# welcomyou/sherpa-vietnamese-asr

Hardware: AMD Instinct MI355X
Metric: audio-sec/sec (xRT) Zipformer-68M offline decode (higher is better)
Workload: dtype bf16; 1 GPU; zipformer-68m greedy_search, batched planner chunks, 1 h per GPU; model=zipformer-68m, weights=greedy-calibrated, chunks_per_gpu=121, batch_pipeline=True, encoder_frames_per_gpu=98813

## Files before the change

include/zasr.h:

```cpp
#ifndef ZASR_H_
#define ZASR_H_

#include <stdint.h>

#ifdef __cplusplus
extern "C" {
#endif

typedef struct zasr_recognizer zasr_recognizer;
typedef struct zasr_result zasr_result;

enum {
  ZASR_OK = 0,
  ZASR_ERR_INVALID = 1,
  ZASR_ERR_NOT_FOUND = 2,
  ZASR_ERR_RUNTIME = 3,
};

enum {
  ZASR_PRECISION_FP32 = 0,
  ZASR_PRECISION_BF16 = 1,
  ZASR_PRECISION_BF16_ENC = 2,
  ZASR_PRECISION_BF16X3 = 3,
  ZASR_PRECISION_BF16X6 = 4,
// ... 107 lines not shown
int zasr_vad_probs(zasr_vad* h, const float* audio, const int64_t* offsets,
                   const int64_t* lengths, int32_t n_files, int32_t auto_boost, float* probs);
int zasr_vad_probs_device(zasr_vad* h, const float* d_audio, const int64_t* offsets,
                          const int64_t* lengths, int32_t n_files, int32_t auto_boost,
                          float* d_probs, void* stream);
int32_t zasr_vad_last_passes(const zasr_vad* h);
int zasr_vad_window(zasr_vad* h, const float* input, const float* state, int32_t n, float* prob,
                    float* state_out);

int32_t zasr_vocab_size(const zasr_recognizer* h);
int32_t zasr_joiner_dim(const zasr_recognizer* h);
int zasr_model_routes(zasr_recognizer* h, char* buf, int64_t cap);
int zasr_fbank_set_mel_banks(zasr_recognizer* h, const float* banks, int32_t n_bins);
int zasr_selftest_launch(int32_t block_threads);
int zasr_selftest_gemm_h3r(int32_t M, int32_t K, int32_t N, int32_t epi, const float* A,
                           const float* W, const float* bias, float* C);
int zasr_selftest_ffn_h3(int32_t R, int32_t D, int32_t F, const float* Y, const float* W1,
                         const float* b1, const float* W2, const float* b2,
                         const float* byp_orig, const float* byp_scale, float* X);
int zasr_selftest_ffn_bf16(int32_t R, int32_t D, int32_t F, const float* W1, const float* b1,
                           const float* W2, const float* b2, const float* byp_orig,
                           const float* byp_scale, float* X, int32_t form);
int zasr_selftest_ffn_bf16_oop(int32_t R, int32_t D, int32_t F, const float* W1, const float* b1,
                               const float* W2, const float* b2, const float* byp_orig,
                               const float* byp_scale, float* X, float* Xout, int32_t form);
int zasr_selftest_ffn_h3_oop(int32_t R, int32_t D, int32_t F, const float* W1, const float* b1,
                             const float* W2, const float* b2, const float* byp_orig,
                             const float* byp_scale, float* X, float* Xout);
int zasr_selftest_seam(int32_t nseq, const int32_t* L, int32_t d, int32_t ds, int32_t dn,
                       int32_t ds_next, int32_t c0, int32_t ldo, const float* xd,
                       const float* orig, const float* s, const float* wn8, const float* wo2,
                       float* next, float* xnext, float* out, float* next_ref, float* xnext_ref,
                       float* out_ref);
int zasr_selftest_attn_block_map(const int32_t* lens, int32_t nseq, int32_t units_per_seq,
                                 int32_t order, uint32_t* out, int64_t cap, int32_t* grid);

int zasr_profile_enable(zasr_recognizer* h, int32_t on);
int zasr_profile_reset(zasr_recognizer* h);
int zasr_profile_report(zasr_recognizer* h, char* buf, int64_t cap);

const char* zasr_last_error(void);
const char* zasr_version(void);

#ifdef __cplusplus
}
#endif
#endif
```

sherpa-vietnamese-asr_amd/csrc/engine.cpp:

```cpp
#include "engine.h"

#include <algorithm>
#include <cmath>
#include <cstring>
#include <deque>
#include <numeric>
#include <cstdlib>
#include <sstream>

#include "common.h"
#include "gemm.h"
#include "host_io.h"
#include "onnx_io.h"

namespace zasr {

namespace {
struct HwNode {
  int tok = -1;
  double tok_score = 0, node_score = 0, out_score = 0;
  bool is_end = false;
  std::vector<std::pair<int, int>> kids;
  int fail = 0, out = -1;
  int child(int t) const {
// ... 583 lines not shown
        for (DLin* l : {&L.na_in, &L.na_out}) mk(*l);
        for (int a = 0; a < 2; ++a)
          for (DLin* l : {&L.sa_in[a], &L.sa_out[a], &L.cv_in[a], &L.cv_out[a]}) mk(*l);
        for (int a = 0; a < 3; ++a)
          for (DLin* l : {&L.ff_in[a], &L.ff_out[a]}) mk(*l);
      }
    ZASR_HIP_CHECK(hipStreamSynchronize(stream_));
    for (DLin* l : {&model_.pw1, &model_.pw2}) {
      std::vector<__bf16> h((size_t)l->N * l->K), pk(h.size());
      ZASR_HIP_CHECK(hipMemcpy(h.data(), l->wh, h.size() * 2, hipMemcpyDeviceToHost));
      pack_frag32_host(h.data(), l->N, l->K, pk.data());
      void* p = nullptr;
      ZASR_HIP_CHECK(hipMalloc(&p, pk.size() * 2));
      model_.allocations.push_back(p);
      ZASR_HIP_CHECK(hipMemcpy(p, pk.data(), pk.size() * 2, hipMemcpyHostToDevice));
      l->wp = p;
    }
    for (auto& s : model_.stacks)
      for (auto& L : s.layers)
        for (int a = 0; a < 3; ++a) {
          const int F = L.ff_in[a].N, d = L.ff_in[a].K;
          if (d < 256 || !ffn_fused_supported(d) || F % 32 != 0 || F > 2048) continue;
          for (DLin* l : {&L.ff_in[a], &L.ff_out[a]}) {
            std::vector<__bf16> h((size_t)l->N * l->K), pk(h.size());
            ZASR_HIP_CHECK(hipMemcpy(h.data(), l->wh, h.size() * 2, hipMemcpyDeviceToHost));
            ffn_pack_host(h.data(), l->N, l->K, pk.data());
            void* p = nullptr;
            ZASR_HIP_CHECK(hipMalloc(&p, pk.size() * 2));
            model_.allocations.push_back(p);
            ZASR_HIP_CHECK(hipMemcpy(p, pk.data(), pk.size() * 2, hipMemcpyHostToDevice));
            l->wp = p;
          }
        }
  }
  {
    const double gb = (double)cfg.V * cfg.V * cfg.joiner_dim * 4.0 / 1e9;
    double max_gb = 24.0;
    if (const char* e = getenv("ZASR_DEC_TABLE_MAX_GB")) max_gb = atof(e);
    if (gb <= max_gb) {
      void* p = nullptr;
      ZASR_HIP_CHECK(hipMalloc(&p, (size_t)cfg.V * cfg.V * cfg.joiner_dim * sizeof(float)));
      model_.allocations.push_back(p);
      model_.dec_table = reinterpret_cast<float*>(p);
      DecoderW dw{model_.dec_tap0, model_.dec_tap1, model_.dec_proj.b, cfg.joiner_dim};
      launch_dec_table(dw, model_.dec_proj.w, cfg.V, model_.dec_table, stream_);
      ZASR_HIP_CHECK(hipStreamSynchronize(stream_));
    }
  }

  {
    std::vector<double> tw(512);
    for (int j = 0; j < 256; ++j) {
      double a = -2.0 * M_PI * j / 512.0;
      tw[2 * j] = std::cos(a);
      tw[2 * j + 1] = std::sin(a);
    }
    ZASR_HIP_CHECK(hipMalloc(&d_twiddle_, 512 * sizeof(double)));
    ZASR_HIP_CHECK(hipMemcpy(d_twiddle_, tw.data(), 512 * sizeof(double), hipMemcpyHostToDevice));
    std::vector<float> win(400);
    for (int i = 0; i < 400; ++i)
      win[i] = (float)std::pow(0.5 - 0.5 * std::cos(2.0 * M_PI / 399.0 * i), 0.85);
    d_window_ = dev(win.data(), 400);
    auto mel = [](float f) { return 1127.0f * logf(1.0f + f / 700.0f); };
    const float mlo = mel(20.0f), mhi = mel(7600.0f);
    const float delta = (mhi - mlo) / 81.0f;
    std::vector<float> banks(80 * 256, 0.f);
// ... 427 lines not shown
      a.v = vv;
      a.out = oa;
      a.map = bm.heads;
      a.map_len = bm.n_heads;
      prof_begin("attn_apply");
      launch_attn_flash(a, k == 0 ? 1 : 2, st_);
      prof_end();
      linear_h(Ly.sa_out[k], oa, true, 12 * h, R, X, false, d, EPI_RESADD);
      return;
    }
    float* vv = ws<float>("ly_vv", (size_t)R * 12 * h);
    float* oa = ws<float>("ly_oa", (size_t)R * 12 * h);
    linear(Ly.sa_in[k], X, d, R, vv, 12 * h, EPI_NONE);
    if (np) {
      AttnFlashArgs a = fa;
      a.v = vv;
      a.out = oa;
      a.map = bm.heads;
      a.map_len = bm.n_heads;
      prof_begin("attn_apply");
      launch_attn_flash(a, k == 0 ? 1 : 2, st_);
      prof_end();
      linear(Ly.sa_out[k], oa, 12 * h, R, X, d, EPI_RESADD);
      return;
    }
    AttnSAArgs sa{qkp, h, Ly.pos_tab, model_.pmax, d_off, B, maxL, stats, vv, oa, stats};
    prof_begin("attn_apply");
    launch_attn_sa(sa, k == 0, false, st_);
    prof_end();
    linear(Ly.sa_out[k], oa, 12 * h, R, X, d, EPI_RESADD);
  };
  auto conv = [&](int k) {
    if (Ly.cv_in[k].wh) {
      __bf16* dc = ws<__bf16>("ly_dc_h", (size_t)R * d);
      if (Ly.cv_in[k].glu) {
        __bf16* g = ws<__bf16>("ly_glu_h", (size_t)R * d);
        linear_h(Ly.cv_in[k], X, false, d, R, g, true, d, EPI_GLU);
        prof_begin("dwconv1d");
        launch_dwconv1d_post_glu_bf16(g, d_off, d_map, R, d, S.K, Ly.cv_dw_w[k], Ly.cv_dw_b[k], dc, st_);
        prof_end();
      } else {
        __bf16* g2 = ws<__bf16>("ly_g2_h", (size_t)R * 2 * d);
        linear_h(Ly.cv_in[k], X, false, d, R, g2, true, 2 * d, EPI_NONE);
        prof_begin("dwconv1d");
        launch_glu_dwconv1d_bf16(g2, d_off, d_map, R, d, S.K, Ly.cv_dw_w[k], Ly.cv_dw_b[k], dc, st_);
        prof_end();
      }
      linear_h(Ly.cv_out[k], dc, true, d, R, X, false, d, EPI_RESADD);
      return;
    }
    float* dc = ws<float>("ly_dc", (size_t)R * d);
    if (Ly.cv_in[k].glu) {
      float* g = ws<float>("ly_glu", (size_t)R * d);
      linear(Ly.cv_in[k], X, d, R, g, d, EPI_GLU);
      prof_begin("dwconv1d");
      launch_dwconv1d_post_glu(g, d_off, d_map, R, d, S.K, Ly.cv_dw_w[k], Ly.cv_dw_b[k], dc, st_);
      prof_end();
    } else {
      float* g2 = ws<float>("ly_g2", (size_t)R * 2 * d);
      linear(Ly.cv_in[k], X, d, R, g2, 2 * d, EPI_NONE);
      prof_begin("dwconv1d");
      launch_glu_dwconv1d(g2, d_off, d_map, R, d, S.K, Ly.cv_dw_w[k], Ly.cv_dw_b[k], dc, st_);
      prof_end();
    }
    linear(Ly.cv_out[k], dc, d, R, X, d, EPI_RESADD);
  };
// ... 1084 lines not shown
```

sherpa-vietnamese-asr_amd/csrc/kernels.h:

```cpp
#pragma once
#include <cstdint>
#include <vector>

#include <hip/hip_runtime.h>

namespace zasr {

struct FbankTables {
  const double* twiddle;
  const float* window;
  const int* mel_start;
  const int* mel_len;
  const int* mel_woff;
  const float* mel_w;
};
void launch_fbank(const float* wav, const long* wav_off, const int* nsamp, const int* fr_off,
                  int nseq, int total_frames, const FbankTables& tabs, float* out,
                  hipStream_t st, bool campp = false);

void launch_silence_flags(const float* wav, long n, int frame_len, float threshold,
                          unsigned char* flags, hipStream_t st);

void launch_selftest_noop(int block_threads);
void selftest_gemm_h3r(int M, int K, int N, int epi, const float* A, const float* W,
// ... 101 lines not shown
                  int total_rows, const float* w , const float* b, void* out,
                  bool out_bf16, hipStream_t st, bool fast = false);
void pack_frag32_host(const __bf16* w, int rows, int cols, __bf16* out);
void launch_convnext_bf16(const void* x, const int* L_off, const int* L_map, int total_rows,
                          const float* dw_w, const float* dw_b, const void* w1, const float* b1,
                          const void* w2, const float* b2, void* ytmp, void* out,
                          hipStream_t st);
void launch_convnext_mlp_h3(const float* y, const float* x, long npos, const void* w1p,
                            const float* b1, const void* w2p, const float* b2, float* out,
                            hipStream_t st);
void launch_dwconv2d_tiled(const float* x, const int* L_off, const int* L_map, int total_rows,
                           const float* w, const float* b, float* out, hipStream_t st);

void selftest_seam(int nseq, const int* L, int d, int ds, int dn, int ds_next, int c0, int ldo,
                   const float* xd, const float* orig, const float* s, const float* wn8,
                   const float* wo2, float* next, float* xnext, float* out, float* next_ref,
                   float* xnext_ref, float* out_ref);
void launch_bias_norm(float* x, int rows, int d, const float* bias, float log_scale,
                      const float* orig, const float* bypass_scale, hipStream_t st,
                      float* copy_out = nullptr);
void launch_bypass(float* x, const float* orig, const float* s, long rows, int d, hipStream_t st);
void launch_glu(const float* x2, float* g, long rows, int d, hipStream_t st);
void launch_dwconv1d_post_glu(const float* g, const int* off, const int* map, int total_rows,
                              int d, int K, const float* w, const float* b, float* out,
                              hipStream_t st);
void launch_dwconv1d_post_glu_bf16(const void* g, const int* off, const int* map,
                                   int total_rows, int d, int K, const float* w, const float* b,
                                   void* out, hipStream_t st);
void launch_glu_dwconv1d(const float* x2, const int* off, const int* map, int total_rows, int d,
                         int K, const float* w, const float* b, float* out, hipStream_t st);
void launch_glu_dwconv1d_bf16(const void* x2, const int* off, const int* map, int total_rows,
                              int d, int K, const float* w, const float* b, void* out,
                              hipStream_t st);
void launch_nonlin_prep(const float* h3, float* t1, long rows, int hid, hipStream_t st);
void launch_downsample(const float* x, const int* off_in, const int* off_out, const int* map_out,
                       int total_out, int d, int ds, const float* w_host8, float* out,
                       hipStream_t st);
void launch_upsample_combine(const float* xd, const float* orig, const int* off_in,
                             const int* off_ds, const int* map_in, int total_rows, int d, int ds,
                             const float* s, float* y, hipStream_t st);
void launch_stack_glue(const float* xd, const float* orig, const int* off_in, const int* off_ds,
                       const int* map_in, int rows, int d, int ds, const float* s, float* next,
                       int dn, float* full, int ldf, int c0, hipStream_t st);
struct SeamDesc {
  const float* xd = nullptr;
  const float* orig = nullptr;
  const float* s = nullptr;
  const int* off_in = nullptr;
  const int* off_ds = nullptr;
  const int* off_run = nullptr;
  const int* map_run = nullptr;
  int runs = 0;
  int rows = 0;
  int d = 0, ds = 1;
  float* next = nullptr;
  int dn = 0;
  int ds_next = 1;
  float* xnext = nullptr;
  const float* wn_host8 = nullptr;
  float* out = nullptr;
  const int* off_out = nullptr;
  const float* wo_host2 = nullptr;
  int ldo = 0, c0 = 0;
};
void launch_seam(const SeamDesc& s, hipStream_t st);
void launch_row2seq(const int* off, int nseq, int total, int* map, hipStream_t st);
// ... 230 lines not shown
```

sherpa-vietnamese-asr_amd/csrc/selftest.cpp:

```cpp
#include <cstring>
#include <memory>
#include <vector>

#include "common.h"
#include "gemm.h"
#include "kernels.h"

namespace zasr {
namespace {
struct DevBuf {
  void* p = nullptr;
  explicit DevBuf(size_t bytes) { ZASR_HIP_CHECK(hipMalloc(&p, bytes > 0 ? bytes : 4)); }
  ~DevBuf() { (void)hipFree(p); }
  template <class T>
  T* as() const { return reinterpret_cast<T*>(p); }
};
void up(DevBuf& d, const void* h, size_t bytes) {
  if (bytes) ZASR_HIP_CHECK(hipMemcpy(d.p, h, bytes, hipMemcpyHostToDevice));
}
}

void selftest_gemm_h3r(int M, int K, int N, int epi, const float* A, const float* W,
                       const float* bias, float* C) {
  ZASR_REQUIRE(M >= 1, "selftest gemm_h3r: M >= 1");
// ... 160 lines not shown
    sd.wn_host8 = wn8;
  }
  if (has_out) {
    sd.out = dout.as<float>();
    sd.off_out = dO.as<int>();
    sd.wo_host2 = wo2;
    sd.ldo = ldo;
    sd.c0 = c0;
  }
  launch_seam(sd, nullptr);
  launch_stack_glue(dxd.as<float>(), dorig.as<float>(), dL.as<int>(), dS.as<int>(), mL.as<int>(),
                    rows, d, ds, ds_.as<float>(), dn > 0 ? dnext_r.as<float>() : nullptr, dn,
                    has_out ? dfull.as<float>() : nullptr, ldo, c0, nullptr);
  if (has_x)
    launch_downsample(dnext_r.as<float>(), dL.as<int>(), dN.as<int>(), mN.as<int>(), rn, dn,
                      ds_next, wn8, dxn_r.as<float>(), nullptr);
  if (has_out)
    launch_downsample(dfull.as<float>(), dL.as<int>(), dO.as<int>(), mO.as<int>(), ro, ldo, 2, wo2,
                      dout_r.as<float>(), nullptr);
  ZASR_HIP_CHECK(hipDeviceSynchronize());
  auto down = [](void* h, const DevBuf& dv, size_t bytes) {
    if (bytes) ZASR_HIP_CHECK(hipMemcpy(h, dv.p, bytes, hipMemcpyDeviceToHost));
  };
  down(next, dnext, bn);
  down(next_ref, dnext_r, bn);
  if (has_x) {
    down(xnext, dxn, bxn);
    down(xnext_ref, dxn_r, bxn);
  }
  down(out, dout, bout);
  down(out_ref, dout_r, bout);
}

}
```

sherpa-vietnamese-asr_amd/csrc/zasr_api.cpp:

```cpp
#include <cstdio>
#include <cstring>
#include <fstream>
#include <memory>
#include <mutex>
#include <sstream>
#include <string>
#include <vector>

#include "../../include/zasr.h"
#include "campp.h"
#include "common.h"
#include "vad.h"
#include "vibert.h"
#include "engine.h"
#include "host_io.h"
#include "onnx_io.h"

using zasr::Engine;
using zasr::TokenResult;

struct zasr_recognizer {
  std::unique_ptr<Engine> eng;
  std::string model_dir;
  std::string tokens_path;
// ... 660 lines not shown
                               const float* byp_scale, float* X, float* Xout, int32_t form) {
  if (!W1 || !b1 || !W2 || !b2 || !X || !Xout) return fail(ZASR_ERR_INVALID, "null argument");
  return guarded([&]() {
    zasr::selftest_ffn_bf16(R, D, F, W1, b1, W2, b2, byp_orig, byp_scale, X, form, Xout);
    return (int)ZASR_OK;
  });
}

int zasr_selftest_ffn_h3_oop(int32_t R, int32_t D, int32_t F, const float* W1, const float* b1,
                             const float* W2, const float* b2, const float* byp_orig,
                             const float* byp_scale, float* X, float* Xout) {
  if (!W1 || !b1 || !W2 || !b2 || !X || !Xout) return fail(ZASR_ERR_INVALID, "null argument");
  return guarded([&]() {
    zasr::selftest_ffn_h3(R, D, F, nullptr, W1, b1, W2, b2, byp_orig, byp_scale, X, Xout);
    return (int)ZASR_OK;
  });
}

int zasr_selftest_seam(int32_t nseq, const int32_t* L, int32_t d, int32_t ds, int32_t dn,
                       int32_t ds_next, int32_t c0, int32_t ldo, const float* xd,
                       const float* orig, const float* s, const float* wn8, const float* wo2,
                       float* next, float* xnext, float* out, float* next_ref, float* xnext_ref,
                       float* out_ref) {
  if (!L || !orig || !wn8 || !wo2 || !next || !xnext || !out || !next_ref || !xnext_ref ||
      !out_ref || (ds > 1 && (!xd || !s)))
    return fail(ZASR_ERR_INVALID, "null argument");
  return guarded([&]() {
    zasr::selftest_seam(nseq, L, d, ds, dn, ds_next, c0, ldo, xd, orig, s, wn8, wo2, next, xnext,
                        out, next_ref, xnext_ref, out_ref);
    return (int)ZASR_OK;
  });
}

int zasr_selftest_attn_block_map(const int32_t* lens, int32_t nseq, int32_t units_per_seq,
                                 int32_t order, uint32_t* out, int64_t cap, int32_t* grid) {
  if (!lens || !grid || (cap > 0 && !out) || cap < 0) return fail(ZASR_ERR_INVALID, "null argument");
  return guarded([&]() {
    std::vector<unsigned> map;
    *grid = zasr::build_attn_block_map(lens, nseq, units_per_seq, order, map);
    if ((int64_t)map.size() > cap) return fail(ZASR_ERR_INVALID, "block map buffer too small");
    std::copy(map.begin(), map.end(), out);
    return (int)ZASR_OK;
  });
}

int zasr_silence_flags(const float* d_wav, int64_t n, int32_t frame_len, float threshold,
                       uint8_t* d_flags, void* stream) {
  if (n < 0 || (n > 0 && (!d_wav || !d_flags))) return fail(ZASR_ERR_INVALID, "null argument");
  return guarded([&]() {
    zasr::launch_silence_flags(d_wav, (long)n, (int)frame_len, threshold, d_flags,
                               reinterpret_cast<hipStream_t>(stream));
    return (int)ZASR_OK;
  });
}

int zasr_set_tokens(zasr_recognizer* h, const char* tokens_path) {
  if (!h || !tokens_path) return fail(ZASR_ERR_INVALID, "null argument");
  return guarded([&]() {
    std::ifstream f(tokens_path);
    if (!f) return fail(ZASR_ERR_NOT_FOUND, std::string("tokens file not found: ") + tokens_path);
    std::lock_guard<std::mutex> lk(h->sym_mu);
    h->tokens_path = tokens_path;
    h->syms.reset();
    return (int)ZASR_OK;
  });
}
// ... 100 lines not shown
```

sherpa-vietnamese-asr_amd/zasr/binding.py:

```python
from __future__ import annotations

import ctypes as C
import dataclasses
import os
from typing import List, Optional, Sequence

import numpy as np

_PKG = os.path.dirname(os.path.dirname(os.path.abspath(__file__)))
DEFAULT_LIB = os.path.join(_PKG, "lib", "libzasr.so")

EXPORTS = (
    "zasr_create", "zasr_destroy", "zasr_convert_model", "zasr_convert_stage_model", "zasr_fbank", "zasr_decode_batch", "zasr_decode_features",
    "zasr_decode_device", "zasr_decode_device_batches", "zasr_encode_features", "zasr_search_encoder_out",
    "zasr_result_count", "zasr_result_num_tokens", "zasr_result_num_frames",
    "zasr_result_tokens", "zasr_result_frames", "zasr_result_log_probs",
    "zasr_result_token_stats", "zasr_result_free", "zasr_vocab_size", "zasr_joiner_dim",
    "zasr_profile_enable", "zasr_profile_reset", "zasr_profile_report", "zasr_last_error",
    "zasr_version", "zasr_campp_create", "zasr_campp_destroy", "zasr_campp_embedding_dim",
    "zasr_campp_fbank", "zasr_campp_embed", "zasr_campp_embed_device", "zasr_campp_windows_device",
    "zasr_vibert_create", "zasr_vibert_destroy", "zasr_vibert_num_labels",
    "zasr_vibert_num_detect", "zasr_vibert_run",
    "zasr_vad_create", "zasr_vad_destroy", "zasr_vad_probs", "zasr_vad_probs_device",
    "zasr_vad_window", "zasr_vad_last_passes", "zasr_silence_flags",
    "zasr_create_stream", "zasr_destroy_stream", "zasr_stream_accept_waveform",
    "zasr_decode_stream", "zasr_decode_streams", "zasr_stream_is_decoded",
    "zasr_stream_num_tokens", "zasr_stream_num_frames", "zasr_stream_tokens",
    "zasr_stream_frames", "zasr_stream_log_probs", "zasr_stream_token_stats",
    "zasr_stream_result_json", "zasr_set_tokens", "zasr_model_routes",
    "zasr_fbank_set_mel_banks", "zasr_selftest_launch", "zasr_decode_host_batches",
    "zasr_selftest_gemm_h3r", "zasr_selftest_ffn_h3", "zasr_selftest_ffn_bf16",
    "zasr_selftest_attn_block_map", "zasr_selftest_seam", "zasr_selftest_ffn_bf16_oop",
    "zasr_selftest_ffn_h3_oop",
)


PRECISIONS = {"fp32": 0, "bf16": 1, "bf16_enc": 2, "bf16x3": 3, "bf16x6": 4, "f16x3": 5}


C_FP = C.POINTER(C.c_float)


class ZasrError(RuntimeError):
    pass


class _Config(C.Structure):
    _fields_ = [
        ("model_dir", C.c_char_p),
        ("decoding_method", C.c_char_p),
        ("max_active_paths", C.c_int32),
        ("blank_penalty", C.c_float),
        ("hotword_tokens", C.POINTER(C.c_int32)),
        ("hotword_lens", C.POINTER(C.c_int32)),
        ("hotword_scores", C.POINTER(C.c_float)),
        ("num_hotwords", C.c_int32),
        ("device_id", C.c_int32),
        ("precision", C.c_int32),
    ]


_lib = None


def load_library(path: Optional[str] = None) -> C.CDLL:
    global _lib
# ... 121 lines not shown
    lib.zasr_stream_tokens.argtypes = [P]
    lib.zasr_stream_tokens.restype = C.POINTER(I32)
    lib.zasr_stream_frames.argtypes = [P]
    lib.zasr_stream_frames.restype = C.POINTER(I32)
    lib.zasr_stream_log_probs.argtypes = [P]
    lib.zasr_stream_log_probs.restype = C.POINTER(C.c_double)
    lib.zasr_stream_token_stats.argtypes = [P]
    lib.zasr_stream_token_stats.restype = fp
    lib.zasr_stream_result_json.argtypes = [P, C.c_char_p, I64, C.POINTER(I64)]
    lib.zasr_stream_result_json.restype = C.c_int
    lib.zasr_set_tokens.argtypes = [P, C.c_char_p]
    lib.zasr_set_tokens.restype = C.c_int
    lib.zasr_model_routes.argtypes = [P, C.c_char_p, I64]
    lib.zasr_model_routes.restype = C.c_int
    lib.zasr_fbank_set_mel_banks.argtypes = [P, fp, I32]
    lib.zasr_fbank_set_mel_banks.restype = C.c_int
    lib.zasr_selftest_launch.argtypes = [I32]
    lib.zasr_selftest_launch.restype = C.c_int
    lib.zasr_selftest_gemm_h3r.argtypes = [I32, I32, I32, I32, fp, fp, fp, fp]
    lib.zasr_selftest_gemm_h3r.restype = C.c_int
    lib.zasr_selftest_ffn_h3.argtypes = [I32, I32, I32, fp, fp, fp, fp, fp, fp, fp, fp]
    lib.zasr_selftest_ffn_h3.restype = C.c_int
    lib.zasr_selftest_ffn_bf16.argtypes = [I32, I32, I32, fp, fp, fp, fp, fp, fp, fp, I32]
    lib.zasr_selftest_ffn_bf16.restype = C.c_int
    lib.zasr_selftest_attn_block_map.argtypes = [C.POINTER(I32), I32, I32, I32,
                                                 C.POINTER(C.c_uint32), I64, C.POINTER(I32)]
    lib.zasr_selftest_attn_block_map.restype = C.c_int
    lib.zasr_selftest_seam.argtypes = [I32, C.POINTER(I32)] + [I32] * 6 + [fp] * 11
    lib.zasr_selftest_seam.restype = C.c_int
    lib.zasr_selftest_ffn_bf16_oop.argtypes = [I32, I32, I32] + [fp] * 8 + [I32]
    lib.zasr_selftest_ffn_bf16_oop.restype = C.c_int
    lib.zasr_selftest_ffn_h3_oop.argtypes = [I32, I32, I32] + [fp] * 8
    lib.zasr_selftest_ffn_h3_oop.restype = C.c_int
    if path is None:
        _lib = lib
    return lib


def convert_model(model_dir: str, out_dir: str, lib_path: Optional[str] = None) -> None:
    lib = load_library(lib_path)
    os.makedirs(out_dir, exist_ok=True)
    rc = lib.zasr_convert_model(model_dir.encode(), out_dir.encode())
    if rc != 0:
        msg = lib.zasr_last_error().decode()
        if rc == 2:
            raise FileNotFoundError(msg)
        raise ZasrError(msg)


def convert_stage_model(kind: str, model_dir: str, out_dir: str,
                        lib_path: Optional[str] = None) -> None:
    lib = load_library(lib_path)
    os.makedirs(out_dir, exist_ok=True)
    rc = lib.zasr_convert_stage_model(kind.encode(), model_dir.encode(), out_dir.encode())
    if rc != 0:
        msg = lib.zasr_last_error().decode()
        if rc == 2:
            raise FileNotFoundError(msg)
        raise ZasrError(msg)


def selftest_launch(block_threads: int, lib_path: Optional[str] = None) -> None:
    lib = load_library(lib_path)
    rc = lib.zasr_selftest_launch(int(block_threads))
    if rc != 0:
        raise ZasrError(lib.zasr_last_error().decode())
# ... 70 lines not shown
            p(out))
    if kind == "bf16":
        rc = lib.zasr_selftest_ffn_bf16_oop(*args, int(form))
    elif kind == "h3":
        rc = lib.zasr_selftest_ffn_h3_oop(*args)
    else:
        raise ValueError(kind)
    if rc != 0:
        raise ZasrError(lib.zasr_last_error().decode())
    return out, X


def selftest_seam(L, d: int, ds: int, dn: int, ds_next: int, c0: int, ldo: int, xd, orig, s,
                  wn8, wo2, fill: float = -777.25, lib_path: Optional[str] = None) -> dict:
    lib = load_library(lib_path)
    L = np.ascontiguousarray(L, dtype=np.int32)
    orig, wn8, wo2 = _f32(orig), _f32(wn8), _f32(wo2)
    xd = None if xd is None else _f32(xd)
    s = None if s is None else _f32(s)
    rows = int(L.sum())
    rn = int(((L + ds_next - 1) // ds_next).sum())
    ro = int(((L + 1) // 2).sum())
    assert orig.shape == (rows, d) and wn8.shape == (8,) and wo2.shape == (2,)
    assert ds == 1 or (xd.shape == (int(((L + ds - 1) // ds).sum()), d) and s.shape == (d,))
    res = {}
    for name, shape in (("next", (rows, dn)), ("xnext", (rn, dn)), ("out", (ro, ldo))):
        for k in (name, name + "_ref"):
            res[k] = np.full(shape, fill, dtype=np.float32)
    p = lambda x: None if x is None else x.ctypes.data_as(C_FP)
    rc = lib.zasr_selftest_seam(len(L), L.ctypes.data_as(C.POINTER(C.c_int32)), int(d), int(ds),
                                int(dn), int(ds_next), int(c0), int(ldo), p(xd), p(orig), p(s),
                                p(wn8), p(wo2), p(res["next"]), p(res["xnext"]), p(res["out"]),
                                p(res["next_ref"]), p(res["xnext_ref"]), p(res["out_ref"]))
    if rc != 0:
        raise ZasrError(lib.zasr_last_error().decode())
    return res


def silence_flags(d_wav_ptr: int, n: int, frame_len: int, threshold: float, d_flags_ptr: int,
                  stream: int = 0, lib_path: Optional[str] = None) -> None:
    lib = load_library(lib_path)
    rc = lib.zasr_silence_flags(C.c_void_p(d_wav_ptr), int(n), int(frame_len),
                                float(threshold), C.c_void_p(d_flags_ptr), C.c_void_p(stream))
    if rc != 0:
        raise ZasrError(lib.zasr_last_error().decode())


@dataclasses.dataclass
class SearchResult:
    token_ids: np.ndarray
    frames: np.ndarray
    log_probs: np.ndarray
    stats: np.ndarray
    T: int


def _f32(a) -> np.ndarray:
    return np.ascontiguousarray(np.asarray(a, dtype=np.float32))


def _ptr_array(arrs: Sequence[np.ndarray]):
    fp = C.POINTER(C.c_float)
    return (fp * len(arrs))(*[a.ctypes.data_as(fp) for a in arrs])


class Recognizer:
# ... 431 lines not shown
```

Measured before the change: 134,800 audio-sec/sec.

## Fuse depthwise conv, SwooshR and conv output GEMM into one conv-tail kernel

Adds a kernel that computes the depthwise 1D convolution with SwooshR activation per 64-row tile in LDS, then immediately feeds that tile to MFMA to do the output projection with bias and residual add into X. This removes the round trip of writing and re-reading the intermediate bf16 activation, along with one kernel launch per conv module. It is enabled only for d=192, K=31 layers that use the GLU input path, with output weights repacked into MFMA fragment order at load. The cost is a more complex kernel with boundary masking across sequence edges and possibly lower occupancy than the tuned standalone GEMM.

Result: no change. 135,400 audio-sec/sec (median of 6 runs) (+0.5%).

```diff
diff --git a/include/zasr.h b/include/zasr.h
--- a/include/zasr.h
+++ b/include/zasr.h
@@ -163,6 +163,11 @@
                        const float* orig, const float* s, const float* wn8, const float* wo2,
                        float* next, float* xnext, float* out, float* next_ref, float* xnext_ref,
                        float* out_ref);
+int zasr_selftest_conv_tail(int32_t nseq, const int32_t* lens, int32_t d, int32_t K,
+                            const float* g, const float* dw_w, const float* dw_b, const float* W,
+                            const float* b, const float* X_in, float* X_pair_out,
+                            float* X_fused_out, int32_t pad_rows, float* g_after);
+int zasr_conv_tail_supported(int32_t d, int32_t K);
 int zasr_selftest_attn_block_map(const int32_t* lens, int32_t nseq, int32_t units_per_seq,
                                  int32_t order, uint32_t* out, int64_t cap, int32_t* grid);
 
diff --git a/sherpa-vietnamese-asr_amd/csrc/conv_tail.hip b/sherpa-vietnamese-asr_amd/csrc/conv_tail.hip
--- /dev/null
+++ b/sherpa-vietnamese-asr_amd/csrc/conv_tail.hip
@@ -0,0 +1,293 @@
+#include "common.h"
+#include "gemm_dev.h"
+#include "kernels.h"
+
+namespace zasr {
+
+namespace {
+
+constexpr int kCtRows = 64;
+constexpr int kCtLdc = 72;
+constexpr int kCtLde = 40;
+
+__device__ __forceinline__ void ct_lds_barrier() {
+  asm volatile("s_waitcnt lgkmcnt(0)" ::: "memory");
+  __builtin_amdgcn_s_barrier();
+}
+
+template <int D, int K>
+__global__ __launch_bounds__(256, 2) void conv_tail_kernel(
+    const __bf16* __restrict__ g, const int* __restrict__ off, const int* __restrict__ map,
+    int total_rows, const float* __restrict__ w, const float* __restrict__ bias,
+    const __bf16* __restrict__ Wp, const float* __restrict__ b_out, float* __restrict__ X) {
+  constexpr int half = K / 2;
+  constexpr int nrows = kCtRows + K - 1;
+  constexpr int NG = D / 64;
+  constexpr int nvec = nrows * 8;
+  constexpr int kIt = (nvec + 255) / 256;
+  constexpr int nw4 = 16 * K;
+  constexpr int kWIt = (nw4 + 255) / 256;
+  static_assert(kWIt <= 2, "conv_tail: two tap vectors per thread");
+  constexpr int WM = D == 192 ? 2 : 1, WN = 4 / WM;
+  constexpr int WTM = kCtRows / WM, WTN = D / WN;
+  constexpr int FM = WTM / 32, FN = WTN / 32;
+  static_assert(D % 64 == 0 && WTN % 32 == 0 && FM >= 1 && FN >= 1, "conv_tail: tile split");
+  constexpr int WH = FN >= 3 ? 2 : 4;
+  static_assert(WH == 2 || WH == 4, "conv_tail: one or two fragment batches per chunk");
+  constexpr int NF = FM * FN;
+  constexpr int PD = NF < 4 ? NF : 4;
+  constexpr int tileB = nrows * 64 * 2;
+  constexpr int epiB = 4 * 32 * kCtLde * 4;
+  constexpr int tileBytes = 2 * tileB > epiB ? 2 * tileB : epiB;
+  __shared__ __attribute__((aligned(16))) unsigned char tileRaw[tileBytes];
+  __shared__ __attribute__((aligned(16))) float sW[2][64 * K];
+  __shared__ __attribute__((aligned(16))) __bf16 sDC[2][kCtRows * kCtLdc];
+  __shared__ int sLo[kCtRows], sHi[kCtRows], sMasked;
+  unsigned short* const tile16 = reinterpret_cast<unsigned short*>(tileRaw);
+
+  const int r0 = xcd_tile(blockIdx.x, gridDim.x) * kCtRows;
+  const int tid = threadIdx.x, lane = tid & 63, wid = tid >> 6;
+  const int wm = wid / WN, wn = wid - wm * WN;
+  const int c = lane;
+  if (tid == 0) sMasked = 0;
+
+  bf16x8 gv[kIt];
+  float4 wv0, wv1;
+  float bnext;
+  auto gload = [&](int gi) {
+    const int c0 = gi * 64;
+#pragma unroll
+    for (int q = 0; q < kIt; ++q) {
+      const int e = tid + 256 * q;
+      const int c8 = e & 7, rr = e >> 3;
+      int r = r0 - half + rr;
+      r = r < 0 ? 0 : (r >= total_rows ? total_rows - 1 : r);
+      gv[q] = *reinterpret_cast<const bf16x8*>(g + (long)r * D + c0 + 8 * c8);
+    }
+    const float4* w4 = reinterpret_cast<const float4*>(w + (long)c0 * K);
+    wv0 = w4[tid < nw4 ? tid : nw4 - 1];
+    if constexpr (kWIt > 1) wv1 = w4[tid + 256 < nw4 ? tid + 256 : nw4 - 1];
+    bnext = bias[c0 + c];
+  };
+  auto sstore = [&](int buf) {
+    unsigned short* t = tile16 + buf * (nrows * 64);
+#pragma unroll
+    for (int q = 0; q < kIt; ++q) {
+      const int e = tid + 256 * q;
+      const int c8 = e & 7, rr = e >> 3;
+      const int r = r0 - half + rr;
+      bf16x8 v = gv[q];
+      if (r < 0 || r >= total_rows) {
+#pragma unroll
+        for (int j = 0; j < 8; ++j) v[j] = (__bf16)0.f;
+      }
+      if (e < nvec) *reinterpret_cast<bf16x8*>(&t[rr * 64 + 8 * c8]) = v;
+    }
+    if (tid < nw4) *reinterpret_cast<float4*>(&sW[buf][4 * tid]) = wv0;
+    if constexpr (kWIt > 1) {
+      if (tid + 256 < nw4) *reinterpret_cast<float4*>(&sW[buf][4 * (tid + 256)]) = wv1;
+    }
+  };
+
+  gload(0);
+  int seq_lo = 0, seq_hi = 0;
+  if (tid < kCtRows && r0 + tid < total_rows) {
+    const int b = map[r0 + tid];
+    seq_lo = off[b];
+    seq_hi = off[b + 1];
+  }
+  sstore(0);
+  float bc = bnext;
+  if (tid < kCtRows) {
+    const int r = r0 + tid;
+    int lo = -half, hi = half;
+    if (r < total_rows) {
+      lo = max(seq_lo - r, -half);
+      hi = min(seq_hi - 1 - r, half);
+    }
+    sLo[tid] = lo;
+    sHi[tid] = hi;
+    if (lo != -half || hi != half) atomicOr(&sMasked, 1);
+  }
+  __syncthreads();
+  const bool masked = sMasked != 0;
+  const int tr0 = wid * 16;
+
+  f32x16 acc[FM][FN];
+#pragma unroll
+  for (int i = 0; i < FM; ++i)
+#pragma unroll
+    for (int j = 0; j < FN; ++j)
+#pragma unroll
+      for (int r = 0; r < 16; ++r) acc[i][j][r] = 0.f;
+
+  const bf16x8* Wf = reinterpret_cast<const bf16x8*>(Wp) + (long)(wn * FN) * (D / 16) * 64 + lane;
+  bf16x8 bw[WH][FN];
+  auto wload = [&](int ks0) {
+#pragma unroll
+    for (int s = 0; s < WH; ++s)
+#pragma unroll
+      for (int j = 0; j < FN; ++j) bw[s][j] = Wf[((long)j * (D / 16) + ks0 + s) * 64];
+  };
+  auto mma = [&](const __bf16* dc, int s0) {
+#pragma unroll
+    for (int s = 0; s < WH; ++s) {
+      bf16x8 a[FM];
+#pragma unroll
+      for (int i = 0; i < FM; ++i)
+        a[i] = *reinterpret_cast<const bf16x8*>(
+            &dc[(wm * WTM + i * 32 + (lane & 31)) * kCtLdc + (s0 + s) * 16 + 8 * (lane >> 5)]);
+#pragma unroll
+      for (int i = 0; i < FM; ++i)
+#pragma unroll
+        for (int j = 0; j < FN; ++j)
+          acc[i][j] = __builtin_amdgcn_mfma_f32_32x32x16_bf16(a[i], bw[s][j], acc[i][j], 0, 0, 0);
+    }
+  };
+
+  for (int gi = 0; gi < NG; ++gi) {
+    const int buf = gi & 1;
+    gload(gi + 1 < NG ? gi + 1 : NG - 1);
+    wload(gi * 4);
+    const unsigned short* t = tile16 + buf * (nrows * 64);
+    auto tv = [&](int rr) {
+      return __builtin_bit_cast(float, (unsigned)t[(tr0 + rr) * 64 + c] << 16);
+    };
+    float wr[K];
+#pragma unroll
+    for (int k = 0; k < K; ++k) wr[k] = sW[buf][c * K + k];
+    float cacc[16];
+#pragma unroll
+    for (int i = 0; i < 16; ++i) cacc[i] = bc;
+    if (!masked) {
+#pragma unroll
+      for (int rr = 0; rr < 16 + K - 1; ++rr) {
+        const float v = tv(rr);
+#pragma unroll
+        for (int i = 0; i < 16; ++i) {
+          const int k = rr - i;
+          if (k >= 0 && k < K) cacc[i] = fmaf(wr[k], v, cacc[i]);
+        }
+      }
+    } else {
+      int lo[16], hi[16];
+#pragma unroll
+      for (int i = 0; i < 16; ++i) {
+        lo[i] = __builtin_amdgcn_readfirstlane(sLo[tr0 + i]);
+        hi[i] = __builtin_amdgcn_readfirstlane(sHi[tr0 + i]);
+      }
+#pragma unroll
+      for (int rr = 0; rr < 16 + K - 1; ++rr) {
+        const float v = tv(rr);
+#pragma unroll
+        for (int i = 0; i < 16; ++i) {
+          const int k = rr - i;
+          if (k >= 0 && k < K && k - half >= lo[i] && k - half <= hi[i])
+            cacc[i] = fmaf(wr[k], v, cacc[i]);
+        }
+      }
+    }
+    __bf16* dc = sDC[buf];
+#pragma unroll
+    for (int i = 0; i < 16; ++i) dc[(tr0 + i) * kCtLdc + c] = (__bf16)swooshr_fast(cacc[i]);
+    if (gi + 1 < NG) {
+      sstore(buf ^ 1);
+      bc = bnext;
+    }
+    ct_lds_barrier();
+    mma(dc, 0);
+    if constexpr (WH < 4) {
+      wload(gi * 4 + WH);
+      mma(dc, WH);
+    }
+  }
+  asm volatile("s_waitcnt vmcnt(0)" ::: "memory");
+
+  float* sE = reinterpret_cast<float*>(tileRaw) + wid * (32 * kCtLde);
+  const int c4 = lane & 7;
+  auto xload = [&](int f, float4 (&pre)[4]) {
+    const int i = f / FN, j = f - i * FN;
+    const int col = wn * WTN + j * 32 + 4 * c4;
+#pragma unroll
+    for (int q = 0; q < 4; ++q) {
+      const int row = r0 + wm * WTM + i * 32 + (lane >> 3) + 8 * q;
+      pre[q] = *reinterpret_cast<const float4*>(
+          X + (long)(row < total_rows ? row : total_rows - 1) * D + col);
+    }
+  };
+  float4 pre[PD][4];
+#pragma unroll
+  for (int f = 0; f < PD; ++f) xload(f, pre[f]);
+#pragma unroll
+  for (int f = 0; f < NF; ++f) {
+    const int i = f / FN, j = f - i * FN;
+#pragma unroll
+    for (int r = 0; r < 16; ++r)
+      sE[((r & 3) + 8 * (r >> 2) + 4 * (lane >> 5)) * kCtLde + (lane & 31)] = acc[i][j][r];
+    __builtin_amdgcn_wave_barrier();
+    const int col = wn * WTN + j * 32 + 4 * c4;
+    float4 bo = make_float4(0.f, 0.f, 0.f, 0.f);
+    if (b_out) bo = *reinterpret_cast<const float4*>(b_out + col);
+    float4 o[4];
+#pragma unroll
+    for (int q = 0; q < 4; ++q) o[q] = pre[f % PD][q];
+    if (f + PD < NF) xload(f + PD, pre[f % PD]);
+#pragma unroll
+    for (int q = 0; q < 4; ++q) {
+      const int rl = (lane >> 3) + 8 * q;
+      const int row = r0 + wm * WTM + i * 32 + rl;
+      float4 v = *reinterpret_cast<const float4*>(&sE[rl * kCtLde + 4 * c4]);
+      if (row < total_rows) {
+        v.x = fmaf(v.x, 1.f, bo.x) + o[q].x;
+        v.y = fmaf(v.y, 1.f, bo.y) + o[q].y;
+        v.z = fmaf(v.z, 1.f, bo.z) + o[q].z;
+        v.w = fmaf(v.w, 1.f, bo.w) + o[q].w;
+        *reinterpret_cast<float4*>(X + (long)row * D + col) = v;
+      }
+    }
+    __builtin_amdgcn_wave_barrier();
+  }
+}
+
+}
+
+bool conv_tail_instantiated(int d, int K) {
+  return (K == 31 && (d == 192 || d == 256)) || (K == 15 && (d == 256 || d == 384 || d == 512));
+}
+
+bool conv_tail_supported(int d, int K) { return d == 192 && K == 31; }
+
+void conv_tail_pack_host(const __bf16* w, int d, __bf16* out) {
+  for (int nf = 0; nf < d / 32; ++nf)
+    for (int ks = 0; ks < d / 16; ++ks)
+      for (int l = 0; l < 64; ++l)
+        for (int j = 0; j < 8; ++j)
+          out[(((size_t)nf * (d / 16) + ks) * 64 + l) * 8 + j] =
+              w[(size_t)(32 * nf + (l & 31)) * d + 16 * ks + 8 * (l >> 5) + j];
+}
+
+void launch_conv_tail(const void* g, const int* off, const int* map, int total_rows, int d, int Kr,
+                      const float* dw_w, const float* dw_b, const void* W_out_packed,
+                      const float* b_out, float* X, hipStream_t st) {
+  if (total_rows <= 0) return;
+  ZASR_REQUIRE(conv_tail_instantiated(d, Kr), "conv_tail: no kernel for (channels, kernel size)");
+  ZASR_REQUIRE((reinterpret_cast<uintptr_t>(g) & 15) == 0 && (reinterpret_cast<uintptr_t>(dw_w) & 15) == 0 &&
+                   (reinterpret_cast<uintptr_t>(W_out_packed) & 15) == 0 &&
+                   (reinterpret_cast<uintptr_t>(X) & 15) == 0 &&
+                   (b_out == nullptr || (reinterpret_cast<uintptr_t>(b_out) & 15) == 0),
+               "conv_tail: operands must be 16-byte aligned");
+  const __bf16* gh = reinterpret_cast<const __bf16*>(g);
+  const __bf16* wp = reinterpret_cast<const __bf16*>(W_out_packed);
+  const dim3 grid(cdiv(total_rows, kCtRows));
+#define ZASR_CT(D_, K_)                                                                      \
+  ZASR_LAUNCH((conv_tail_kernel<D_, K_>), grid, dim3(256), 0, st, gh, off, map, total_rows, \
+              dw_w, dw_b, wp, b_out, X)
+  if (d == 192) ZASR_CT(192, 31);
+  else if (d == 256 && Kr == 31) ZASR_CT(256, 31);
+  else if (d == 256) ZASR_CT(256, 15);
+  else if (d == 384) ZASR_CT(384, 15);
+  else ZASR_CT(512, 15);
+#undef ZASR_CT
+}
+
+}
diff --git a/sherpa-vietnamese-asr_amd/csrc/engine.cpp b/sherpa-vietnamese-asr_amd/csrc/engine.cpp
--- a/sherpa-vietnamese-asr_amd/csrc/engine.cpp
+++ b/sherpa-vietnamese-asr_amd/csrc/engine.cpp
@@ -639,6 +639,20 @@
             l->wp = p;
           }
         }
+    for (auto& s : model_.stacks)
+      for (auto& L : s.layers)
+        for (int a = 0; a < 2; ++a) {
+          DLin& l = L.cv_out[a];
+          if (!L.cv_in[a].glu || l.N != s.d || l.K != s.d || !conv_tail_supported(s.d, s.K)) continue;
+          std::vector<__bf16> h((size_t)l.N * l.K), pk(h.size());
+          ZASR_HIP_CHECK(hipMemcpy(h.data(), l.wh, h.size() * 2, hipMemcpyDeviceToHost));
+          conv_tail_pack_host(h.data(), s.d, pk.data());
+          void* p = nullptr;
+          ZASR_HIP_CHECK(hipMalloc(&p, pk.size() * 2));
+          model_.allocations.push_back(p);
+          ZASR_HIP_CHECK(hipMemcpy(p, pk.data(), pk.size() * 2, hipMemcpyHostToDevice));
+          l.wp = p;
+        }
   }
   {
     const double gb = (double)cfg.V * cfg.V * cfg.joiner_dim * 4.0 / 1e9;
@@ -1132,6 +1146,19 @@
   };
   auto conv = [&](int k) {
     if (Ly.cv_in[k].wh) {
+      if (Ly.cv_in[k].glu && Ly.cv_out[k].wp) {
+        const DLin& lo = Ly.cv_out[k];
+        __bf16* g = ws<__bf16>("ly_glu_h", (size_t)R * d);
+        linear_h(Ly.cv_in[k], X, false, d, R, g, true, d, EPI_GLU);
+        if (prof_shapes_ && prof_on_)
+          prof_begin(shape_key("enc_gemm", R, d, d, true, true, false, EPI_RESADD));
+        else
+          prof_begin("enc_gemm");
+        launch_conv_tail(g, d_off, d_map, R, d, S.K, Ly.cv_dw_w[k], Ly.cv_dw_b[k], lo.wp,
+                         lo.bh ? lo.bh : lo.b, X, st_);
+        prof_end();
+        return;
+      }
       __bf16* dc = ws<__bf16>("ly_dc_h", (size_t)R * d);
       if (Ly.cv_in[k].glu) {
         __bf16* g = ws<__bf16>("ly_glu_h", (size_t)R * d);
diff --git a/sherpa-vietnamese-asr_amd/csrc/kernels.h b/sherpa-vietnamese-asr_amd/csrc/kernels.h
--- a/sherpa-vietnamese-asr_amd/csrc/kernels.h
+++ b/sherpa-vietnamese-asr_amd/csrc/kernels.h
@@ -157,6 +157,15 @@
 void launch_glu_dwconv1d_bf16(const void* x2, const int* off, const int* map, int total_rows,
                               int d, int K, const float* w, const float* b, void* out,
                               hipStream_t st);
+bool conv_tail_instantiated(int d, int K);
+bool conv_tail_supported(int d, int K);
+void conv_tail_pack_host(const __bf16* w, int d, __bf16* out);
+void launch_conv_tail(const void* g, const int* off, const int* map, int total_rows, int d, int Kr,
+                      const float* dw_w, const float* dw_b, const void* W_out_packed,
+                      const float* b_out, float* X, hipStream_t st);
+void selftest_conv_tail(int nseq, const int* lens, int d, int K, int pad_rows, const float* g,
+                        const float* dw_w, const float* dw_b, const float* W, const float* b,
+                        const float* X_in, float* X_pair_out, float* X_fused_out, float* g_after);
 void launch_nonlin_prep(const float* h3, float* t1, long rows, int hid, hipStream_t st);
 void launch_downsample(const float* x, const int* off_in, const int* off_out, const int* map_out,
                        int total_out, int d, int ds, const float* w_host8, float* out,
diff --git a/sherpa-vietnamese-asr_amd/csrc/selftest.cpp b/sherpa-vietnamese-asr_amd/csrc/selftest.cpp
--- a/sherpa-vietnamese-asr_amd/csrc/selftest.cpp
+++ b/sherpa-vietnamese-asr_amd/csrc/selftest.cpp
@@ -216,4 +216,57 @@
   down(out_ref, dout_r, bout);
 }
 
-}
+void selftest_conv_tail(int nseq, const int* lens, int d, int K, int pad_rows, const float* g,
+                        const float* dw_w, const float* dw_b, const float* W, const float* b,
+                        const float* X_in, float* X_pair_out, float* X_fused_out, float* g_after) {
+  ZASR_REQUIRE(nseq >= 1 && pad_rows >= 0, "selftest conv_tail: sizes");
+  ZASR_REQUIRE(conv_tail_instantiated(d, K), "selftest conv_tail: no kernel for (channels, kernel size)");
+  std::vector<int> off(nseq + 1, 0);
+  for (int s = 0; s < nseq; ++s) {
+    ZASR_REQUIRE(lens[s] >= 1, "selftest conv_tail: every sequence needs a row");
+    off[s + 1] = off[s] + lens[s];
+  }
+  const int R = off[nseq];
+  const size_t n = (size_t)R * d, nx = (size_t)(R + pad_rows) * d, nw = (size_t)d * d;
+  std::vector<__bf16> gh(n), wh(nw), wpk(nw);
+  for (size_t i = 0; i < n; ++i) gh[i] = (__bf16)g[i];
+  for (size_t i = 0; i < nw; ++i) wh[i] = (__bf16)W[i];
+  conv_tail_pack_host(wh.data(), d, wpk.data());
+  DevBuf dOff((size_t)(nseq + 1) * 4), dMap((size_t)R * 4), dG(n * 2), dDc(n * 2), dWd((size_t)d * K * 4),
+      dBd((size_t)d * 4), dWh(nw * 2), dWp(nw * 2), dB((size_t)d * 4), dXp(nx * 4), dXf(nx * 4);
+  up(dOff, off.data(), (size_t)(nseq + 1) * 4);
+  launch_row2seq(dOff.as<int>(), nseq, R, dMap.as<int>(), nullptr);
+  up(dG, gh.data(), n * 2);
+  up(dWd, dw_w, (size_t)d * K * 4);
+  up(dBd, dw_b, (size_t)d * 4);
+  up(dWh, wh.data(), nw * 2);
+  up(dWp, wpk.data(), nw * 2);
+  if (b) up(dB, b, (size_t)d * 4);
+  up(dXp, X_in, nx * 4);
+  up(dXf, X_in, nx * 4);
+  launch_dwconv1d_post_glu_bf16(dG.p, dOff.as<int>(), dMap.as<int>(), R, d, K, dWd.as<float>(),
+                                dBd.as<float>(), dDc.p, nullptr);
+  GemmParams p{};
+  p.A = dDc.as<float>();
+  p.lda = d;
+  p.sbk = 1;
+  p.sbn = d;
+  p.C = dXp.as<float>();
+  p.ldc = d;
+  p.bias = b ? dB.as<float>() : nullptr;
+  p.M = R;
+  p.N = d;
+  p.K = d;
+  p.alpha = 1.f;
+  p.max_M = R;
+  gemm_bf16(p, dWh.p, EPI_RESADD, ALOAD_DENSE, nullptr, true, false);
+  launch_conv_tail(dG.p, dOff.as<int>(), dMap.as<int>(), R, d, K, dWd.as<float>(), dBd.as<float>(),
+                   dWp.p, b ? dB.as<float>() : nullptr, dXf.as<float>(), nullptr);
+  ZASR_HIP_CHECK(hipDeviceSynchronize());
+  ZASR_HIP_CHECK(hipMemcpy(X_pair_out, dXp.p, nx * 4, hipMemcpyDeviceToHost));
+  ZASR_HIP_CHECK(hipMemcpy(X_fused_out, dXf.p, nx * 4, hipMemcpyDeviceToHost));
+  ZASR_HIP_CHECK(hipMemcpy(gh.data(), dG.p, n * 2, hipMemcpyDeviceToHost));
+  for (size_t i = 0; i < n; ++i) g_after[i] = (float)gh[i];
+}
+
+}
diff --git a/sherpa-vietnamese-asr_amd/csrc/zasr_api.cpp b/sherpa-vietnamese-asr_amd/csrc/zasr_api.cpp
--- a/sherpa-vietnamese-asr_amd/csrc/zasr_api.cpp
+++ b/sherpa-vietnamese-asr_amd/csrc/zasr_api.cpp
@@ -716,6 +716,21 @@
   });
 }
 
+int zasr_selftest_conv_tail(int32_t nseq, const int32_t* lens, int32_t d, int32_t K,
+                            const float* g, const float* dw_w, const float* dw_b, const float* W,
+                            const float* b, const float* X_in, float* X_pair_out,
+                            float* X_fused_out, int32_t pad_rows, float* g_after) {
+  if (!lens || !g || !dw_w || !dw_b || !W || !X_in || !X_pair_out || !X_fused_out || !g_after)
+    return fail(ZASR_ERR_INVALID, "null argument");
+  return guarded([&]() {
+    zasr::selftest_conv_tail(nseq, lens, d, K, pad_rows, g, dw_w, dw_b, W, b, X_in, X_pair_out,
+                             X_fused_out, g_after);
+    return (int)ZASR_OK;
+  });
+}
+
+int zasr_conv_tail_supported(int32_t d, int32_t K) { return zasr::conv_tail_supported(d, K) ? 1 : 0; }
+
 int zasr_selftest_attn_block_map(const int32_t* lens, int32_t nseq, int32_t units_per_seq,
                                  int32_t order, uint32_t* out, int64_t cap, int32_t* grid) {
   if (!lens || !grid || (cap > 0 && !out) || cap < 0) return fail(ZASR_ERR_INVALID, "null argument");
diff --git a/sherpa-vietnamese-asr_amd/zasr/binding.py b/sherpa-vietnamese-asr_amd/zasr/binding.py
--- a/sherpa-vietnamese-asr_amd/zasr/binding.py
+++ b/sherpa-vietnamese-asr_amd/zasr/binding.py
@@ -31,7 +31,7 @@
     "zasr_fbank_set_mel_banks", "zasr_selftest_launch", "zasr_decode_host_batches",
     "zasr_selftest_gemm_h3r", "zasr_selftest_ffn_h3", "zasr_selftest_ffn_bf16",
     "zasr_selftest_attn_block_map", "zasr_selftest_seam", "zasr_selftest_ffn_bf16_oop",
-    "zasr_selftest_ffn_h3_oop",
+    "zasr_selftest_ffn_h3_oop", "zasr_selftest_conv_tail", "zasr_conv_tail_supported",
 )
 
 
@@ -219,6 +219,10 @@
     lib.zasr_selftest_ffn_bf16_oop.restype = C.c_int
     lib.zasr_selftest_ffn_h3_oop.argtypes = [I32, I32, I32] + [fp] * 8
     lib.zasr_selftest_ffn_h3_oop.restype = C.c_int
+    lib.zasr_selftest_conv_tail.argtypes = [I32, C.POINTER(I32), I32, I32] + [fp] * 8 + [I32, fp]
+    lib.zasr_selftest_conv_tail.restype = C.c_int
+    lib.zasr_conv_tail_supported.argtypes = [I32, I32]
+    lib.zasr_conv_tail_supported.restype = C.c_int
     if path is None:
         _lib = lib
     return lib
@@ -355,6 +359,31 @@
                                 int(dn), int(ds_next), int(c0), int(ldo), p(xd), p(orig), p(s),
                                 p(wn8), p(wo2), p(res["next"]), p(res["xnext"]), p(res["out"]),
                                 p(res["next_ref"]), p(res["xnext_ref"]), p(res["out_ref"]))
+    if rc != 0:
+        raise ZasrError(lib.zasr_last_error().decode())
+    return res
+
+
+def conv_tail_supported(d: int, K: int, lib_path: Optional[str] = None) -> bool:
+    return bool(load_library(lib_path).zasr_conv_tail_supported(int(d), int(K)))
+
+
+def selftest_conv_tail(lens, g, dw_w, dw_b, W, b, X, pad_rows: int = 0, fill: float = -777.25,
+                       lib_path: Optional[str] = None) -> dict:
+    lib = load_library(lib_path)
+    lens = np.ascontiguousarray(lens, dtype=np.int32)
+    g, dw_w, dw_b, W, X = (_f32(v) for v in (g, dw_w, dw_b, W, X))
+    b = None if b is None else _f32(b)
+    R, d = g.shape
+    K = dw_w.shape[1]
+    assert R == int(lens.sum()) and X.shape == (R, d) and W.shape == (d, d) and dw_w.shape[0] == d
+    x_in = np.full((R + pad_rows, d), fill, dtype=np.float32)
+    x_in[:R] = X
+    res = {"pair": np.empty_like(x_in), "fused": np.empty_like(x_in), "g_after": np.empty_like(g)}
+    p = lambda x: None if x is None else x.ctypes.data_as(C_FP)
+    rc = lib.zasr_selftest_conv_tail(len(lens), lens.ctypes.data_as(C.POINTER(C.c_int32)), d, K,
+                                     p(g), p(dw_w), p(dw_b), p(W), p(b), p(x_in), p(res["pair"]),
+                                     p(res["fused"]), int(pad_rows), p(res["g_after"]))
     if rc != 0:
         raise ZasrError(lib.zasr_last_error().decode())
     return res
```
